# tomershay100/mp3-steganography-lib

Hardware: AMD Instinct MI355X
Metric: MP3 frames/sec (decode+re-encode) @44.1kHz stereo 128kbps, 1→8 GPU (higher is better)
Workload: dtype f64 (decode) / int32 (encode); 1 GPU; 10000-frame full decode->stego-embed->re-encode pipeline per MI355X (BASELINE configs[2]); MP3 main data + side info resident in HBM, MP3 frames out; the message cursor chain is decided and the serial chains of the rate loop are checked on the device inside every step; frames_per_gpu=10000, channels=2, message_bits=536, chain_verdict_units_to_redo=0, message_variant_entries=1874, parallelism=frames sharded over 1 GPU(s), no collective

## Files before the change

### mp3-steganography-lib_amd/csrc/k_pack.hpp

```cpp
#pragma once

namespace mp3s {

constexpr int PACK_DW = 372;
constexpr int PACK_FAM = 260;
constexpr int PACK_PT_QUAD = 4 * PACK_FAM, PACK_PT_NONE = PACK_PT_QUAD + 32, PACK_PT = PACK_PT_NONE + 1;
#define MP3S_PS_OVERFLOW 1
#define MP3S_PS_BAD_TABLE 2

__device__ __forceinline__ void lds_put(uint32_t *fb, uint32_t pos, uint32_t val, int n)
{
    if (n <= 0) return;
    const uint32_t d = pos >> 5, o = pos & 31;
    const uint64_t w = (uint64_t)val << (64 - o - n);
    atomicOr(&fb[d], (uint32_t)(w >> 32));
    if ((uint32_t)w) atomicOr(&fb[d + 1], (uint32_t)w);
}

__device__ __forceinline__ int pack_wave_sum(int v, bool on) { return (int)wave_add_u32(on ? (uint32_t)v : 0u); }

__global__ __launch_bounds__(256) void k_enc_pack(
    const int16_t *__restrict__ ix, const mp3s_gr_out *__restrict__ gr, const int32_t *__restrict__ en, int n_frames,
    int sri, int bri, int whole_slots, const uint32_t *__restrict__ frame_off, const uint8_t *__restrict__ padding,
    uint8_t *__restrict__ mp3, int32_t *__restrict__ scfsi_out, int32_t *__restrict__ status, int32_t *__restrict__ sync,
    int f_begin )
{
    __shared__ uint32_t fb3[3][PACK_DW];
    __shared__ uint32_t pt[PACK_PT];
    __shared__ int wg_err;
    const int wave0 = __builtin_amdgcn_readfirstlane(threadIdx.x >> 6), lane0 = threadIdx.x & 63;
    for (int i = threadIdx.x; i < 1024; i += 256) {
        const uint32_t len = i < 256 ? c_tab.hlen13[i] : (i < 512 ? c_tab.hlen15[i - 256] : (i < 768 ? c_tab.hlen16[i - 512] : c_tab.hlen24[i - 768]));
        pt[(i >> 8) * PACK_FAM + (i & 255)] = (&c_tab.hcod[0][0])[i] | (len << 24);
    }
    if (threadIdx.x < 16) {
        pt[PACK_PT_QUAD + threadIdx.x] = (uint32_t)c_tab.hcod_c1a[threadIdx.x] | ((uint32_t)c_tab.hlen_c1a[threadIdx.x] << 24);
        pt[PACK_PT_QUAD + 16 + threadIdx.x] = (15u - threadIdx.x) | (4u << 24);
    }
    if (threadIdx.x == 0) pt[PACK_PT_NONE] = 0;
    for (int i = threadIdx.x; i < 3 * PACK_DW; i += 256) (&fb3[0][0])[i] = 0;
    if (threadIdx.x == 0) wg_err = 0;
    __syncthreads();
    int rot = 0;
    for (int f = f_begin + blockIdx.x; f < n_frames; f += gridDim.x) {
    const int lane = lane0, tid = (int)threadIdx.x;
    int lane_p = lane0, wave = wave0;
    asm volatile("" : "+v"(lane_p), "+s"(wave));
    uint32_t *fb = fb3[rot];
    {
        uint32_t *cl = fb3[rot == 2 ? 0 : rot + 1];
        for (int i = tid; i < PACK_DW; i += 256) cl[i] = 0;
    }
    const int pad = padding[f];
    int p23v[4];
    {
        const int bits_per_frame = 8 * (whole_slots + pad);
        const int mean_bits = (bits_per_frame - 288) / 2;
        int sum = 0;
#pragma unroll
        for (int e = 0; e < 4; e++) {
            p23v[e] = __builtin_amdgcn_readfirstlane(gr[((long)f * 2 + (e & 1)) * 2 + (e >> 1)].part2_3_length);
            sum += p23v[e];
        }
        int stuffing = 2 * mean_bits - sum + ((mean_bits & 1) ? 1 : 0);
        if (stuffing < 0) stuffing = 0;
        if (stuffing) {
            if (p23v[0] + stuffing < 4095) p23v[0] += stuffing;
            else
#pragma unroll
                for (int e = 0; e < 4; e++) {
                    const int extra = 4095 - p23v[e], now = extra < stuffing ? extra : stuffing;
                    p23v[e] += now; stuffing -= now;
                }
        }
    }
    const int e = wave, grn = e >> 1, ch = e & 1;
    const long u = ((long)f * 2 + ch) * 2 + grn;
    const mp3s_gr_out &g = gr[u];
    if (wave < 2) {
        const long u0 = ((long)f * 2 + wave) * 2, u1 = u0 + 1;
        int a = 0, tot21 = 0;
        if (lane_p < 22) {
            a = en[u0 * 22 + lane] - en[u1 * 22 + lane];
            a = a < 0 ? -a : a;
        }
        tot21 = __builtin_amdgcn_readlane(a, 21);
        int sc = lane_p < 21 ? a : 0;
        sc += __builtin_amdgcn_update_dpp(0, sc, 0x111, 0xf, 0xf, false);
        sc += __builtin_amdgcn_update_dpp(0, sc, 0x112, 0xf, 0xf, false);
        sc += __builtin_amdgcn_update_dpp(0, sc, 0x114, 0xf, 0xf, false);
        sc += __builtin_amdgcn_update_dpp(0, sc, 0x118, 0xf, 0xf, false);
        const int row0 = __builtin_amdgcn_readlane(sc, 15);
        const int p5 = __builtin_amdgcn_readlane(sc, 5), p10 = __builtin_amdgcn_readlane(sc, 10), q20 = __builtin_amdgcn_readlane(sc, 20);
        const int tp = row0 + q20;
        int cond = 2 + (gr[u0].xrmax != 0) + (gr[u1].xrmax != 0);
        if (tot21 < 10) cond++;
        if (tp < 100) cond++;
        const int band_sum[4] = {p5, p10 - p5, row0 - p10, q20};
        uint32_t scbits = 0;
#pragma unroll
        for (int b = 0; b < 4; b++) {
            const int s0 = band_sum[b];
            const int v = (cond == 6 && s0 < 10) ? 1 : 0;
            scbits = (scbits << 1) | (uint32_t)v;
            if (lane_p == 0) scfsi_out[((long)f * 2 + wave) * 4 + b] = v;
        }
        if (lane_p == 0) {
            lds_put(fb, 44 + 4 * wave, scbits, 4);
            if (wave == 0) {
                const uint32_t h = (0x7ffu << 21) | (3u << 19) | (1u << 17) | (1u << 16) | ((uint32_t)bri << 12) |
                                   ((uint32_t)(sri % 3) << 10) | ((uint32_t)pad << 9) | (1u << 2);
                fb[0] = h;
            }
        }
    }
    if (lane_p < 4) {
        const uint32_t f0 = ((uint32_t)p23v[e] << 9) | (uint32_t)g.big_values;
        const uint32_t f1 = (((uint32_t)(g.quantizer_step + 210) & 0xff) << 5);
        const uint32_t f2 = ((uint32_t)g.table_select[0] << 10) | ((uint32_t)g.table_select[1] << 5) | (uint32_t)g.table_select[2];
        const uint32_t f3 = ((uint32_t)g.region0_count << 6) | ((uint32_t)g.region1_count << 3) | (uint32_t)g.count1table_select;
        const uint32_t v = lane_p == 0 ? f0 : (lane_p == 1 ? f1 : (lane_p == 2 ? f2 : f3));
        const int n = lane_p == 0 ? 21 : (lane_p == 1 ? 13 : (lane_p == 2 ? 15 : 10));
        const uint32_t at = lane_p == 0 ? 0u : (lane_p == 1 ? 21u : (lane_p == 2 ? 34u : 49u));
        lds_put(fb, 52 + 59 * (uint32_t)e + at, v, n);
    }

    const int ts0 = g.table_select[0], ts1 = g.table_select[1], ts2 = g.table_select[2], c1sel = g.count1table_select;
    uint32_t ustart = 288;
#pragma unroll
    for (int k = 0; k < 3; k++) ustart += k < e ? (uint32_t)p23v[k] : 0u;
    const int bv = g.big_values, c1 = g.count1;
    const int32_t *sfb = c_tab.sfb_long[sri];
    const int r1s = sfb[g.region0_count + 1], r2s = sfb[g.region0_count + 1 + g.region1_count + 1];
    int xv[10];
    {
        const uint32_t *xp = reinterpret_cast<const uint32_t *>(ix + u * 576 + lane * 10);
#pragma unroll
        for (int k = 0; k < 5; k++) {
            const uint32_t w = (lane_p * 5 + k) < 288 ? xp[k] : 0u;
            xv[2 * k] = (int)(int16_t)(w & 0xffff); xv[2 * k + 1] = (int)(int16_t)(w >> 16);
        }
    }
    uint32_t c2[6];
#pragma unroll
    for (int k = 0; k < 5; k++) c2[k] = (uint32_t)((xv[2 * k] & 1) | ((xv[2 * k + 1] & 1) << 1));
    c2[5] = (uint32_t)__builtin_amdgcn_update_dpp(0, (int)c2[0], 0x130, 0xf, 0xf, false);
    uint32_t code0[5], code1[5]; int n0[5], n1[5];
    int tot = 0;
    uint32_t Kr[3];
    bool any_bad = false;
    {
        const int tsr[3] = {ts0, ts1, ts2};
#pragma unroll
        for (int r = 0; r < 3; r++) {
            const int ti = tsr[r];
            const int fam = ti == 13 ? 0 : (ti == 15 ? 1 : (ti < 24 ? 2 : 3));
            Kr[r] = ti ? (uint32_t)fam | ((uint32_t)lin_bits_of(ti) << 2) | (1u << 6) : 0u;
            const int lo = r == 0 ? 0 : (r == 1 ? r1s : r2s), hi = r == 0 ? r1s : (r == 1 ? r2s : 576);
            any_bad |= ti != 0 && ti != 13 && ti != 15 && ti < 16 && lo < 2 * bv && lo < hi;
        }
    }
    const uint32_t quad_base = (uint32_t)(PACK_PT_QUAD + (c1sel ? 16 : 0));
#pragma unroll
    for (int k = 0; k < 5; k++) {
        const int p = lane * 5 + k;
        const int vx = xv[2 * k], vy = xv[2 * k + 1];
        const uint32_t x = (uint32_t)(vx < 0 ? -vx : vx), y = (uint32_t)(vy < 0 ? -vy : vy);
        const int i = 2 * p;
        const uint32_t K = i >= r2s ? Kr[2] : (i >= r1s ? Kr[1] : Kr[0]);
        const uint32_t Ke = p < bv ? K : 0u;
        const bool in_c1 = (uint32_t)(p - bv) < (uint32_t)(2 * c1);
        const uint32_t lb = __builtin_amdgcn_ubfe(Ke, 2, 4);
        const uint32_t lbx = x > 14 ? lb : 0u, lby = y > 14 ? lb : 0u;
        const uint32_t nzx = x < 1 ? x : 1u, nzy = y < 1 ? y : 1u;
        uint32_t ext = __builtin_amdgcn_ubfe(x - 15u, 0, lbx);
        ext = (ext << nzx) | ((uint32_t)vx >> 31);
        ext = (ext << lby) | __builtin_amdgcn_ubfe(y - 15u, 0, lby);
        ext = (ext << nzy) | ((uint32_t)vy >> 31);
        const uint32_t xb = lbx + nzx + lby + nzy;
        const bool inside = Ke != 0 || in_c1;
        const uint32_t xx = x > 14 ? 15u : x, yy = y > 14 ? 15u : y;
        const uint32_t q = (c2[k] | (c2[k + 1] << 2)) & 15u;
        const bool quad = in_c1 && !((p - bv) & 1);
        const uint32_t tix = Ke != 0 ? (Ke & 3u) * (uint32_t)PACK_FAM + xx * 16u + yy : (quad ? quad_base + q : (uint32_t)PACK_PT_NONE);
        const uint32_t word = pt[tix];
        code0[k] = word & 0xffffffu;
        n0[k] = (int)(word >> 24);
        code1[k] = inside ? ext : 0u;
        n1[k] = inside ? (int)xb : 0;
        tot += n0[k] + n1[k];
    }
    const int incl = (int)wave_scan_u32((uint32_t)tot);
    const int huff_bits = __builtin_amdgcn_readlane(incl, 63);
    if (tot) {
        const uint32_t pos0 = ustart + (uint32_t)(incl - tot);
        uint32_t d = pos0 >> 5;
        uint32_t cnt = pos0 & 31u;
        uint64_t top = 0;
        auto append = [&](uint32_t v, int n) {
            top |= (uint64_t)v << ((64u - cnt - (uint32_t)n) & 63u);
            cnt += (uint32_t)n;
            atomicOr(&fb[d], (uint32_t)(top >> 32));
            const uint32_t adv = cnt >> 5;
            top <<= 32u * adv; d += adv; cnt &= 31u;
        };
#pragma unroll
        for (int k = 0; k < 5; k++) { append(code0[k], n0[k]); append(code1[k], n1[k]); }
        atomicOr(&fb[d], (uint32_t)(top >> 32));
    }
    const int p23 = e == 0 ? p23v[0] : (e == 1 ? p23v[1] : (e == 2 ? p23v[2] : p23v[3]));
    if (huff_bits > p23 || any_bad) { if (lane_p == 0) atomicOr(&wg_err, any_bad ? MP3S_PS_BAD_TABLE : MP3S_PS_OVERFLOW); }
    else
        for (uint32_t s = ustart + huff_bits + 32u * lane; s < ustart + (uint32_t)p23; s += 64u * 32u) {
            const uint32_t n = (ustart + p23 - s) < 32u ? (ustart + p23 - s) : 32u;
            lds_put(fb, s, n == 32 ? 0xffffffffu : ((1u << n) - 1), (int)n);
        }
    __syncthreads();
    const int nbytes = whole_slots + pad;
    const uint32_t off = frame_off[f];
    auto byte_at = [&](int k) -> uint32_t { return (fb[k >> 2] >> (24 - 8 * (k & 3))) & 0xffu; };
    const int head = (int)((4u - (off & 3u)) & 3u) < nbytes ? (int)((4u - (off & 3u)) & 3u) : nbytes;
    const int n_dw = (nbytes - head) >> 2, tail0 = head + 4 * n_dw;
    if (tid < head) mp3[off + tid] = (uint8_t)byte_at(tid);
    uint32_t *outw = reinterpret_cast<uint32_t *>(mp3 + off + head);
    {
        const int hq = head >> 2, hs = 8 * (head & 3);
        for (int j = tid; j < n_dw; j += 256) {
            const uint32_t hi = fb[hq + j], lo = fb[hq + j + 1];
            const uint32_t be = hs ? __builtin_amdgcn_alignbit(hi, lo, 32 - hs) : hi;
            outw[j] = __builtin_bswap32(be);
        }
    }
    if (tid < nbytes - tail0) mp3[off + tail0 + tid] = (uint8_t)byte_at(tail0 + tid);
    rot = rot == 2 ? 0 : rot + 1;
    }
    __syncthreads();
    if (threadIdx.x != 0) return;
    const int g = wg_err;
    if (!sync) {
        if (g) atomicOr(status, g);
        return;
    }
    unsigned all;
    if (arrive_with_bits(sync, (unsigned)g, gridDim.x, &all)) *status = (int32_t)all;
}

}
```

Measured before the change: 20.14 million frames/s.

## Vectorize Huffman packing with packed 16-bit ops and per-lane region masks

Rewrites the per-lane Huffman code assembly in the pack kernel. It uses packed 16-bit abs/min/sub_sat and udot2 to compute table indices and linbits fields, and replaces per-pair region selects with precomputed 30-bit lane masks and a table-family lookup constant. The side-info write becomes three whole-word atomics from a 64-bit assembled value. The bitstream append now uses an alignbit accumulator that writes only completed words, and stuffing bits are filled with one word-aligned atomic per dword. The aim is to cut VALU and LDS atomic count, in exchange for subtle correctness risks around the clamped loads and the mask boundaries.

```diff
diff --git a/mp3-steganography-lib_amd/csrc/k_pack.hpp b/mp3-steganography-lib_amd/csrc/k_pack.hpp
--- a/mp3-steganography-lib_amd/csrc/k_pack.hpp
+++ b/mp3-steganography-lib_amd/csrc/k_pack.hpp
@@ -15,6 +15,17 @@
     const uint64_t w = (uint64_t)val << (64 - o - n);
     atomicOr(&fb[d], (uint32_t)(w >> 32));
     if ((uint32_t)w) atomicOr(&fb[d + 1], (uint32_t)w);
+}
+
+__device__ __forceinline__ uint32_t pack_bfi(uint32_t mask, uint32_t a, uint32_t b) { return (mask & a) | (~mask & b); }
+
+typedef uint16_t pk_u16 __attribute__((ext_vector_type(2)));
+typedef int16_t pk_i16 __attribute__((ext_vector_type(2)));
+__device__ __forceinline__ pk_u16 pack_pk_min1(pk_u16 a)
+{
+    pk_u16 r;
+    asm("v_pk_min_u16 %0, %1, 1 op_sel_hi:[1,0]" : "=v"(r) : "v"(a));
+    return r;
 }
 
 __device__ __forceinline__ int pack_wave_sum(int v, bool on) { return (int)wave_add_u32(on ? (uint32_t)v : 0u); }
@@ -77,6 +88,7 @@
     const int e = wave, grn = e >> 1, ch = e & 1;
     const long u = ((long)f * 2 + ch) * 2 + grn;
     const mp3s_gr_out &g = gr[u];
+    const int p23 = __builtin_amdgcn_readfirstlane(e == 0 ? p23v[0] : (e == 1 ? p23v[1] : (e == 2 ? p23v[2] : p23v[3])));
     if (wave < 2) {
         const long u0 = ((long)f * 2 + wave) * 2, u1 = u0 + 1;
         int a = 0, tot21 = 0;
@@ -114,107 +126,117 @@
             }
         }
     }
-    if (lane_p < 4) {
-        const uint32_t f0 = ((uint32_t)p23v[e] << 9) | (uint32_t)g.big_values;
+    {
+        const uint32_t f0 = ((uint32_t)p23 << 9) | (uint32_t)g.big_values;
         const uint32_t f1 = (((uint32_t)(g.quantizer_step + 210) & 0xff) << 5);
         const uint32_t f2 = ((uint32_t)g.table_select[0] << 10) | ((uint32_t)g.table_select[1] << 5) | (uint32_t)g.table_select[2];
         const uint32_t f3 = ((uint32_t)g.region0_count << 6) | ((uint32_t)g.region1_count << 3) | (uint32_t)g.count1table_select;
-        const uint32_t v = lane_p == 0 ? f0 : (lane_p == 1 ? f1 : (lane_p == 2 ? f2 : f3));
-        const int n = lane_p == 0 ? 21 : (lane_p == 1 ? 13 : (lane_p == 2 ? 15 : 10));
-        const uint32_t at = lane_p == 0 ? 0u : (lane_p == 1 ? 21u : (lane_p == 2 ? 34u : 49u));
-        lds_put(fb, 52 + 59 * (uint32_t)e + at, v, n);
+        const uint64_t top = ((((uint64_t)f0 << 38) | ((uint64_t)f1 << 25) | ((uint64_t)f2 << 10) | f3)) << 5;
+        const uint32_t at = 52 + 59 * (uint32_t)e, o = at & 31u;
+        const uint64_t d01 = top >> o;
+        const uint32_t d2 = (uint32_t)(((uint64_t)(uint32_t)top << 32) >> o);
+        const uint32_t v = lane_p == 0 ? (uint32_t)(d01 >> 32) : (lane_p == 1 ? (uint32_t)d01 : d2);
+        if (lane_p < 3) atomicOr(&fb[(at >> 5) + (uint32_t)lane], v);
     }
 
     const int ts0 = g.table_select[0], ts1 = g.table_select[1], ts2 = g.table_select[2], c1sel = g.count1table_select;
     uint32_t ustart = 288;
 #pragma unroll
     for (int k = 0; k < 3; k++) ustart += k < e ? (uint32_t)p23v[k] : 0u;
-    const int bv = g.big_values, c1 = g.count1;
+    const int bvr = g.big_values, bv = bvr < 288 ? bvr : 288, c1 = g.count1;
     const int32_t *sfb = c_tab.sfb_long[sri];
     const int r1s = sfb[g.region0_count + 1], r2s = sfb[g.region0_count + 1 + g.region1_count + 1];
-    int xv[10];
-    {
-        const uint32_t *xp = reinterpret_cast<const uint32_t *>(ix + u * 576 + lane * 10);
-#pragma unroll
-        for (int k = 0; k < 5; k++) {
-            const uint32_t w = (lane_p * 5 + k) < 288 ? xp[k] : 0u;
-            xv[2 * k] = (int)(int16_t)(w & 0xffff); xv[2 * k + 1] = (int)(int16_t)(w >> 16);
-        }
-    }
-    uint32_t c2[6];
-#pragma unroll
-    for (int k = 0; k < 5; k++) c2[k] = (uint32_t)((xv[2 * k] & 1) | ((xv[2 * k + 1] & 1) << 1));
-    c2[5] = (uint32_t)__builtin_amdgcn_update_dpp(0, (int)c2[0], 0x130, 0xf, 0xf, false);
+    uint32_t w[5];
+    {
+        const char *xb0 = reinterpret_cast<const char *>(ix + u * 576);
+        const int oa = lane * 20 < 1140 ? lane * 20 : 1140, ob = lane * 20 + 12 < 1144 ? lane * 20 + 12 : 1144;
+        const uint32_t *xa = reinterpret_cast<const uint32_t *>(xb0 + oa), *xc = reinterpret_cast<const uint32_t *>(xb0 + ob);
+        w[0] = xa[0]; w[1] = xa[1]; w[2] = xa[2]; w[3] = xc[0]; w[4] = xc[1];
+    }
+    bool any_bad = false;
+    uint32_t Wr[3], Ur[3];
+    {
+        const int tsr[3] = {ts0, ts1, ts2};
+#pragma unroll
+        for (int r = 0; r < 3; r++) {
+            const int ti = tsr[r];
+            const uint32_t fam = (uint32_t)(0xffffaaaa62aaaaaaull >> (2 * (ti & 31))) & 3u;
+            Wr[r] = (fam | ((uint32_t)lin_bits_of(ti) << 2)) * 0x01041041u;
+            Ur[r] = ti ? 0x3fffffffu : 0u;
+            const int lo = r == 0 ? 0 : (r == 1 ? r1s : r2s), hi = r == 0 ? r1s : (r == 1 ? r2s : 576);
+            any_bad |= ti != 0 && ti != 13 && ti != 15 && ti < 16 && lo < 2 * bvr && lo < hi;
+        }
+    }
+    const int l30 = lane * 30;
+    auto below = [&](int bound) -> uint32_t {
+        const int s = min(max(6 * bound - l30, 0), 30);
+        return (1u << s) - 1u;
+    };
+    const int cend = bv + 2 * c1 < 288 ? bv + 2 * c1 : 288;
+    const uint32_t M1 = below((r1s + 1) >> 1), M2 = below((r2s + 1) >> 1), MB = below(bv), ME = below(cend);
+    const uint32_t P = pack_bfi(M1, Wr[0], pack_bfi(M2, Wr[1], Wr[2]));
+    const uint32_t MU = pack_bfi(M1, Ur[0], pack_bfi(M2, Ur[1], Ur[2]));
+    const uint32_t INS = pack_bfi(MB, MU, ME);
+    const uint32_t odd = 0u - (uint32_t)((lane ^ bv) & 1);
+    const uint32_t quad_base = (uint32_t)(PACK_PT_QUAD + (c1sel ? 16 : 0));
+    const int nb5 = bv - lane * 5;
+#pragma unroll
+    for (int k = 0; k < 5; k++) w[k] &= (uint32_t)__builtin_amdgcn_sbfe((int)INS, 6 * k, 1);
+    uint32_t lowb[6];
+#pragma unroll
+    for (int k = 0; k < 5; k++) lowb[k] = w[k] & 0x00010001u;
+    lowb[5] = (uint32_t)__builtin_amdgcn_update_dpp(0, (int)lowb[0], 0x130, 0xf, 0xf, false);
     uint32_t code0[5], code1[5]; int n0[5], n1[5];
     int tot = 0;
-    uint32_t Kr[3];
-    bool any_bad = false;
-    {
-        const int tsr[3] = {ts0, ts1, ts2};
-#pragma unroll
-        for (int r = 0; r < 3; r++) {
-            const int ti = tsr[r];
-            const int fam = ti == 13 ? 0 : (ti == 15 ? 1 : (ti < 24 ? 2 : 3));
-            Kr[r] = ti ? (uint32_t)fam | ((uint32_t)lin_bits_of(ti) << 2) | (1u << 6) : 0u;
-            const int lo = r == 0 ? 0 : (r == 1 ? r1s : r2s), hi = r == 0 ? r1s : (r == 1 ? r2s : 576);
-            any_bad |= ti != 0 && ti != 13 && ti != 15 && ti < 16 && lo < 2 * bv && lo < hi;
-        }
-    }
-    const uint32_t quad_base = (uint32_t)(PACK_PT_QUAD + (c1sel ? 16 : 0));
 #pragma unroll
     for (int k = 0; k < 5; k++) {
-        const int p = lane * 5 + k;
-        const int vx = xv[2 * k], vy = xv[2 * k + 1];
-        const uint32_t x = (uint32_t)(vx < 0 ? -vx : vx), y = (uint32_t)(vy < 0 ? -vy : vy);
-        const int i = 2 * p;
-        const uint32_t K = i >= r2s ? Kr[2] : (i >= r1s ? Kr[1] : Kr[0]);
-        const uint32_t Ke = p < bv ? K : 0u;
-        const bool in_c1 = (uint32_t)(p - bv) < (uint32_t)(2 * c1);
-        const uint32_t lb = __builtin_amdgcn_ubfe(Ke, 2, 4);
-        const uint32_t lbx = x > 14 ? lb : 0u, lby = y > 14 ? lb : 0u;
-        const uint32_t nzx = x < 1 ? x : 1u, nzy = y < 1 ? y : 1u;
-        uint32_t ext = __builtin_amdgcn_ubfe(x - 15u, 0, lbx);
-        ext = (ext << nzx) | ((uint32_t)vx >> 31);
-        ext = (ext << lby) | __builtin_amdgcn_ubfe(y - 15u, 0, lby);
-        ext = (ext << nzy) | ((uint32_t)vy >> 31);
-        const uint32_t xb = lbx + nzx + lby + nzy;
-        const bool inside = Ke != 0 || in_c1;
-        const uint32_t xx = x > 14 ? 15u : x, yy = y > 14 ? 15u : y;
-        const uint32_t q = (c2[k] | (c2[k + 1] << 2)) & 15u;
-        const bool quad = in_c1 && !((p - bv) & 1);
-        const uint32_t tix = Ke != 0 ? (Ke & 3u) * (uint32_t)PACK_FAM + xx * 16u + yy : (quad ? quad_base + q : (uint32_t)PACK_PT_NONE);
-        const uint32_t word = pt[tix];
+        const uint32_t lb = __builtin_amdgcn_ubfe(P, 6 * k + 2, 4), fam = __builtin_amdgcn_ubfe(P, 6 * k, 2);
+        const pk_u16 c15 = {15, 15};
+        const pk_u16 a = __builtin_bit_cast(pk_u16, __builtin_elementwise_abs(__builtin_bit_cast(pk_i16, w[k])));
+        const pk_u16 cl = __builtin_elementwise_min(a, c15);
+        const pk_u16 nz = pack_pk_min1(a);
+        const pk_u16 lbs = {(uint16_t)lb, (uint16_t)lb};
+        const pk_u16 wid = __builtin_elementwise_sub_sat(lbs, (c15 - cl) * (pk_u16){16, 16}) + nz;
+        const pk_u16 fld = __builtin_elementwise_sub_sat(a, c15) * (pk_u16){2, 2} + (__builtin_bit_cast(pk_u16, w[k]) >> (pk_u16){15, 15});
+        const uint32_t wu = __builtin_bit_cast(uint32_t, wid), fu = __builtin_bit_cast(uint32_t, fld);
+        code1[k] = ((fu & 0xffffu) << (wu >> 16)) | (fu >> 16);
+        n1[k] = (int)((wu & 0xffffu) + (wu >> 16));
+        const uint32_t big = __builtin_amdgcn_udot2(cl, (pk_u16){16, 1}, fam * (uint32_t)PACK_FAM, false);
+        const uint32_t q = __builtin_amdgcn_udot2(__builtin_bit_cast(pk_u16, lowb[k + 1]), (pk_u16){4, 8},
+                                                  __builtin_amdgcn_udot2(__builtin_bit_cast(pk_u16, lowb[k]), (pk_u16){1, 2}, quad_base, false), false);
+        const uint32_t qn = pack_bfi((k & 1) ? ~odd : odd, (uint32_t)PACK_PT_NONE, q);
+        const uint32_t word = pt[k < nb5 ? big : qn] & (uint32_t)__builtin_amdgcn_sbfe((int)INS, 6 * k, 1);
         code0[k] = word & 0xffffffu;
         n0[k] = (int)(word >> 24);
-        code1[k] = inside ? ext : 0u;
-        n1[k] = inside ? (int)xb : 0;
         tot += n0[k] + n1[k];
     }
     const int incl = (int)wave_scan_u32((uint32_t)tot);
     const int huff_bits = __builtin_amdgcn_readlane(incl, 63);
     if (tot) {
-        const uint32_t pos0 = ustart + (uint32_t)(incl - tot);
-        uint32_t d = pos0 >> 5;
-        uint32_t cnt = pos0 & 31u;
-        uint64_t top = 0;
+        uint32_t pos = ustart + (uint32_t)(incl - tot);
+        uint32_t d = pos >> 5;
+        uint64_t acc = 0;
         auto append = [&](uint32_t v, int n) {
-            top |= (uint64_t)v << ((64u - cnt - (uint32_t)n) & 63u);
-            cnt += (uint32_t)n;
-            atomicOr(&fb[d], (uint32_t)(top >> 32));
-            const uint32_t adv = cnt >> 5;
-            top <<= 32u * adv; d += adv; cnt &= 31u;
+            acc = (acc << (uint32_t)n) | v;
+            pos += (uint32_t)n;
+            const uint32_t full = __builtin_amdgcn_alignbit((uint32_t)(acc >> 32), (uint32_t)acc, pos);
+            const uint32_t dn = pos >> 5;
+            atomicOr(&fb[d], dn != d ? full : 0u);
+            d = dn;
         };
 #pragma unroll
         for (int k = 0; k < 5; k++) { append(code0[k], n0[k]); append(code1[k], n1[k]); }
-        atomicOr(&fb[d], (uint32_t)(top >> 32));
-    }
-    const int p23 = e == 0 ? p23v[0] : (e == 1 ? p23v[1] : (e == 2 ? p23v[2] : p23v[3]));
+        atomicOr(&fb[d], __builtin_amdgcn_alignbit((uint32_t)acc, 0u, pos));
+    }
     if (huff_bits > p23 || any_bad) { if (lane_p == 0) atomicOr(&wg_err, any_bad ? MP3S_PS_BAD_TABLE : MP3S_PS_OVERFLOW); }
-    else
-        for (uint32_t s = ustart + huff_bits + 32u * lane; s < ustart + (uint32_t)p23; s += 64u * 32u) {
-            const uint32_t n = (ustart + p23 - s) < 32u ? (ustart + p23 - s) : 32u;
-            lds_put(fb, s, n == 32 ? 0xffffffffu : ((1u << n) - 1), (int)n);
-        }
+    else {
+        const uint32_t s0 = ustart + (uint32_t)huff_bits, s1 = ustart + (uint32_t)p23;
+        for (uint32_t j = (s0 >> 5) + (uint32_t)lane; 32u * j < s1; j += 64u) {
+            const uint32_t a = s0 > 32u * j ? s0 - 32u * j : 0u;
+            const uint32_t b = s1 - 32u * j < 32u ? s1 - 32u * j : 32u;
+            atomicOr(&fb[j], (0xffffffffu >> a) & ~(0x7fffffffu >> (b - 1u)));
+        }
+    }
     __syncthreads();
     const int nbytes = whole_slots + pad;
     const uint32_t off = frame_off[f];
```

After: 20.52 million frames/s (median of 6 runs). 1.9% higher.
